# jhong93/vpd

Hardware: AMD Instinct MI355X
Metric: frame-crops/sec (VPD student train) (higher is better)
Workload: dtype bf16; 1 GPU; configs[1]: Diving48-shaped synthetic crops 128x128, ResNet-34 student (5-ch RGB+flow), emb_dim 128, sum-MSE + AdamW, batch=256 per GPU; global_batch=256, parallelism=dp1

## Files before the change

include/vpd_hip.h:

```cpp
#ifndef VPD_HIP_H
#define VPD_HIP_H
#include <stddef.h>
#ifdef __cplusplus
extern "C" {
#endif

typedef struct vpd_plan vpd_plan_t;

const char* vpd_last_error(void);
int vpd_abi_version(void);
const char* vpd_elem_dtype(void);

int vpd_plan_create(const char* arch, int c_in, int img_h, int img_w, int emb_dim, int motion,
                    int max_batch, int train, vpd_plan_t** out);
#define VPD_TRAIN_EARLY_BUCKET0 2
void vpd_plan_destroy(vpd_plan_t* plan);

int vpd_plan_num_tensors(const vpd_plan_t* plan);
int vpd_plan_tensor_info(const vpd_plan_t* plan, int i, int* kind, int* is_decoder, long long* offset,
                         long long* numel, int* ndim, int dims[4]);
long long vpd_plan_param_numel(const vpd_plan_t* plan);
int vpd_plan_num_bn(const vpd_plan_t* plan);
int vpd_plan_bn_info(const vpd_plan_t* plan, int i, int* channels, long long* rm_off, long long* rv_off);
long long vpd_plan_bn_numel(const vpd_plan_t* plan);
// ... 144 lines not shown
                            const float* gammaA, double* rowsA, void* dzA, float* dgammaA, float* dbetaA, const void* zB,
                            const float* meanB, const float* rstdB, const float* gammaB, double* rowsB, void* dzB,
                            float* dgammaB, float* dbetaB, void* sync, unsigned* err, int n, int H, int W, int C, void* stream);
int vpd_op_bn_backward_residency(int M, int C, int pair, int* out4);
int vpd_op_avgpool(const void* act_padded, int n, int H, int W, int C, int pad, float* pooled, void* stream);
int vpd_op_avgpool_bwd(const float* dpooled, int n, int H, int W, int C, void* dact, void* stream);
int vpd_op_sgemm(const float* A, const float* B, float* Y, const float* bias, int M, int N, int K, int ta, int tb, int relu,
                 void* stream);
int vpd_op_colsum(const float* A, int M, int N, float* out, void* stream);
int vpd_op_relu_mask(float* d, const float* act, long long n, void* stream);
int vpd_op_mse(const float* e, const float* t, long long n, float* de, float* loss_step, double* loss_accum, void* stream);
int vpd_op_wgrad(const void* dz_bf16, const void* x_bf16, float* dw, int n, int dzHp, int dzWp, int dzC, int dzpad,
                 int xHp, int xWp, int xC, int Hs, int Ws, int istr, int Kc, int Co, const int* tapset9,
                 float* slab, void* stream);
size_t vpd_op_wgrad_slab_bytes(void);
int vpd_op_wgrad_pair(const void* dz_bf16, const void* dz2_bf16, const void* x_bf16, float* dw, float* dw2, int n, int dzHp, int dzWp,
                      int dzC, int dzpad, int xHp, int xWp, int xC, int Hs, int Ws, int istr, int Kc, int Co, const int* tapset9,
                      float* slab, float* slab2, void* stream);
int vpd_op_wgrad_pair_lds_bytes(int Hs, int Ws, int ns, long long* bytes);
int vpd_op_tr_read_probe(const void* tile_bf16, void* out_bf16, void* stream);
size_t vpd_op_wgrad128_table_bytes(void);
size_t vpd_op_wgrad128_slab_floats(int Co, int Ci);
int vpd_op_wgrad128_group(int nprob, const void* const* dz, const void* const* x, float* const* dw, float* const* slab,
                          const int* dims, void* dev_table, void* stream);
int vpd_op_wgrad128_schedule(int n, const int* dims4, int G, int* ksplit, int* blk_begin, int* tasks, int cap,
                             double* est_us);

#ifdef __cplusplus
}
#endif
// ... 2 lines not shown
```

vpd_amd/_lib.py:

```python
import ctypes as C
import os

_HERE = os.path.dirname(os.path.abspath(__file__))
LIB_PATH = os.environ.get("VPD_LIB_PATH") or os.path.join(_HERE, "libvpdhip.so")
LIB_PATH_F16 = os.environ.get("VPD_LIB_PATH_F16") or os.path.join(_HERE, "libvpdhip_f16.so")
ABI_VERSION = 5

c_int_p = C.POINTER(C.c_int)
c_ll_p = C.POINTER(C.c_longlong)
vp = C.c_void_p

SIGNATURES = {
    "vpd_last_error": (C.c_char_p, []),
    "vpd_abi_version": (C.c_int, []),
    "vpd_elem_dtype": (C.c_char_p, []),
    "vpd_plan_create": (C.c_int, [C.c_char_p, C.c_int, C.c_int, C.c_int, C.c_int, C.c_int, C.c_int, C.c_int,
                                  C.POINTER(vp)]),
    "vpd_plan_destroy": (None, [vp]),
    "vpd_plan_num_tensors": (C.c_int, [vp]),
    "vpd_plan_tensor_info": (C.c_int, [vp, C.c_int, c_int_p, c_int_p, c_ll_p, c_ll_p, c_int_p, c_int_p]),
    "vpd_plan_param_numel": (C.c_longlong, [vp]),
    "vpd_plan_num_bn": (C.c_int, [vp]),
    "vpd_plan_bn_info": (C.c_int, [vp, C.c_int, c_int_p, c_ll_p, c_ll_p]),
    "vpd_plan_bn_numel": (C.c_longlong, [vp]),
# ... 49 lines not shown
    "vpd_op_conv1x1_bn_dispatch": (C.c_int, [C.c_int] * 6 + [c_int_p]),
    "vpd_op_stem_pool_forward": (C.c_int, [vp] * 5 + [C.c_int] * 5 + [vp]),
    "vpd_op_stem_dgrad": (C.c_int, [vp, vp, vp, C.c_int, C.c_int, C.c_int, C.c_int, vp]),
    "vpd_op_stem_pool_backward": (C.c_int, [vp] * 15 + [C.c_int] * 4 + [vp]),
    "vpd_op_bn_backward": (C.c_int, [vp] * 15 + [C.c_int] + [vp, vp] + [C.c_int] * 6 + [vp]),
    "vpd_op_bn_backward_pair": (C.c_int, [vp] * 20 + [C.c_int] * 4 + [vp]),
    "vpd_op_bn_backward_residency": (C.c_int, [C.c_int, C.c_int, C.c_int, c_int_p]),
    "vpd_op_avgpool": (C.c_int, [vp] + [C.c_int] * 5 + [vp, vp]),
    "vpd_op_avgpool_bwd": (C.c_int, [vp] + [C.c_int] * 4 + [vp, vp]),
    "vpd_op_sgemm": (C.c_int, [vp] * 4 + [C.c_int] * 6 + [vp]),
    "vpd_op_colsum": (C.c_int, [vp, C.c_int, C.c_int, vp, vp]),
    "vpd_op_relu_mask": (C.c_int, [vp, vp, C.c_longlong, vp]),
    "vpd_op_mse": (C.c_int, [vp, vp, C.c_longlong, vp, vp, vp, vp]),
    "vpd_op_wgrad": (C.c_int, [vp, vp, vp] + [C.c_int] * 13 + [c_int_p, vp, vp]),
    "vpd_op_wgrad_slab_bytes": (C.c_size_t, []),
    "vpd_op_wgrad_pair": (C.c_int, [vp] * 5 + [C.c_int] * 13 + [c_int_p, vp, vp, vp]),
    "vpd_op_wgrad_pair_lds_bytes": (C.c_int, [C.c_int, C.c_int, C.c_int, c_ll_p]),
    "vpd_op_tr_read_probe": (C.c_int, [vp, vp, vp]),
    "vpd_op_wgrad128_table_bytes": (C.c_size_t, []),
    "vpd_op_wgrad128_slab_floats": (C.c_size_t, [C.c_int, C.c_int]),
    "vpd_op_wgrad128_group": (C.c_int, [C.c_int, vp, vp, vp, vp, c_int_p, vp, vp]),
    "vpd_op_wgrad128_schedule": (C.c_int, [C.c_int, c_int_p, C.c_int, c_int_p, c_int_p, c_int_p, C.c_int,
                                           C.POINTER(C.c_double)]),
}

_libs = {}


class VpdHipError(RuntimeError):
    pass


def lib(dtype="bf16"):
    if dtype in _libs:
        return _libs[dtype]
    if dtype not in ("bf16", "fp16"):
        raise VpdHipError("unknown element type %r (bf16 | fp16)" % (dtype,))
    path = LIB_PATH if dtype == "bf16" else LIB_PATH_F16
    name = os.path.basename(path)
    if not os.path.isfile(path):
        raise VpdHipError(
            "%s not found at %s: build it with `python -c 'import __graft_entry__ as g; g.build()'` "
            "or `make -C vpd_amd/csrc`.  vpd_amd has no PyTorch/CPU fallback." % (name, path))
    import torch
    h = C.CDLL(path)
    ab_build = "VPD_LIB_PATH" in os.environ and dtype == "bf16"
    for sym, (res, args) in SIGNATURES.items():
        try:
            fn = getattr(h, sym)
        except AttributeError as e:
            if ab_build and (sym.startswith("vpd_op_") or sym in ("vpd_elem_dtype", "vpd_plan_set_loss_scale", "vpd_backward_ext")):
                continue
            raise VpdHipError("%s lacks symbol %s declared in include/vpd_hip.h" % (name, sym)) from e
        fn.restype = res
        fn.argtypes = args
    if h.vpd_abi_version() != ABI_VERSION and not (ab_build and os.environ.get("VPD_LIB_ALLOW_ABI") == str(h.vpd_abi_version())):
        raise VpdHipError("%s ABI version %d != expected %d" % (name, h.vpd_abi_version(), ABI_VERSION))
    if hasattr(h, "vpd_elem_dtype") and h.vpd_elem_dtype().decode() != dtype:
        raise VpdHipError("%s was built with %s elements, %s asked for" % (path, h.vpd_elem_dtype().decode(), dtype))
    _libs[dtype] = h
    return h
# ... 7 lines not shown
```

vpd_amd/csrc/conv_wgrad.hip:

```cpp
#include <string.h>
#include <algorithm>
#include <type_traits>
#include <utility>
#include <vector>
#include "common.h"

typedef const void __attribute__((address_space(1)))* wg_gptr_t;
typedef void __attribute__((address_space(3)))* wg_lptr_t;
typedef const char __attribute__((address_space(3)))* wg_lds_cp;

static __device__ __forceinline__ int wg_f(int r) { return ((r >> 1) & 1) | (((r >> 3) & 1) << 1); }
static __device__ __forceinline__ int wg_swz_off(int r, int col) { return r * 64 + ((((col >> 4) ^ wg_f(r)) << 4) | (col & 15)); }
static __device__ __forceinline__ int wg_src_piece(int r, int piece) { return (((piece >> 1) ^ wg_f(r)) << 1) | (piece & 1); }

static __device__ __forceinline__ bf16x8 wg_tr_read(wg_lds_cp lo_addr, wg_lds_cp hi_addr) {
    typedef s16x4 __attribute__((address_space(3))) * lds_p;
    const s16x4 lo = __builtin_amdgcn_ds_read_tr16_b64_v4i16((lds_p)lo_addr);
    const s16x4 hi = __builtin_amdgcn_ds_read_tr16_b64_v4i16((lds_p)hi_addr);
    s16x8 v;
    v[0] = lo[0]; v[1] = lo[1]; v[2] = lo[2]; v[3] = lo[3];
    v[4] = hi[0]; v[5] = hi[1]; v[6] = hi[2]; v[7] = hi[3];
    return __builtin_bit_cast(bf16x8, v);
}
static __device__ __forceinline__ bf16x8 wg_tr_read(const bf16_t* tile, int o0, int o1) {
// ... 444 lines not shown
    if (i < n4)
        for (int s2 = gi; s2 < ksplit; s2 += groups) {
            const float4 v = slab[(long)s2 * n4 + i];
            a.x += v.x; a.y += v.y; a.z += v.z; a.w += v.w;
        }
    sh[gi][o] = a;
    __syncthreads();
    if (gi == 0 && i < n4) {
        for (int k = 1; k < groups; ++k) {
            const float4 v = sh[k][o];
            a.x += v.x; a.y += v.y; a.z += v.z; a.w += v.w;
        }
        r.dw[pi][i] = a;
    }
}
static void wg_launch_reduce(const WgReduceGroup& red, hipStream_t stream) {
    if (red.nprob < 1) return;
    int max_ks = 1;
    long max_n4 = 0;
    for (int i = 0; i < red.nprob; ++i) {
        max_n4 = red.n4[i] > max_n4 ? red.n4[i] : max_n4;
        max_ks = red.ksplit[i] > max_ks ? red.ksplit[i] : max_ks;
    }
    const int groups = max_ks < 16 ? max_ks : 16;
    hipLaunchKernelGGL(wgrad_slab_reduce_group_kernel, dim3((unsigned)((max_n4 + 63) / 64), red.nprob), dim3(64 * groups), 0, stream,
                       red, groups);
}


template <int R0, int R1>
static __device__ __forceinline__ void wgrad_stem_half(const WgradParams& p, const bf16_t* ring, int STAGE, int nch,
                                                       int ctile, int lane) {
    constexpr int NT = R1 - R0;
    const int W0 = p.Ws, Wp = p.xWp;
    f32x4 acc[NT][4];
#pragma unroll
    for (int t = 0; t < NT; ++t)
#pragma unroll
        for (int a = 0; a < 4; ++a) acc[t][a] = f32x4{0.f, 0.f, 0.f, 0.f};
    const int gq = lane >> 4, i16 = lane & 15, q = i16 >> 2, pp = i16 & 3;
    int offA[4][2], baseB[2][2];
// ... 944 lines not shown
```

vpd_amd/csrc/kernels.h:

```cpp
#pragma once
#include <vector>

#include "common.h"

struct BnApplyParams {
    const bf16_t* z;
    const float* scale; const float* shift;
    int res_kind;
    const bf16_t* res; int rHp, rWp, rpad;
    const float* rscale; const float* rshift;
    bf16_t* out; int oHp, oWp, opad;
    int M, H, W, C, relu;
    unsigned char* mask_out;
    int xcd_tile_px;
};

struct StemPoolParams {
    const bf16_t* z; int Hz, Wz;
    const float* scale; const float* shift;
    bf16_t* out; int opad;
    unsigned char* idx;
    int N, Ho, Wo, C;
};

// ... 52 lines not shown
bool vpd_conv_takes_bn_sums(const ConvParams& p);
struct ConvDispatch {
    int kclass;
    int pws;
    int geo;
    int c64x2;
    int ws1x1, stream1x1;
    int halo;
    int bm, bn;
    int mode;
    int tiles_per_block;
};
ConvDispatch vpd_conv_dispatch(const ConvParams& p);
int vpd_conv_xcd_tile_px(const ConvParams& p);
hipError_t vpd_launch_wgrad_reduce(const WgradParams& p, hipStream_t stream);
extern "C" int vpd_conv_bm(int M, int Co);
hipError_t vpd_launch_wgrad(const WgradParams& p, hipStream_t stream);
size_t vpd_wgrad_slab_bytes();
bool vpd_wgrad_group_eligible(const WgradParams& p);
size_t vpd_wgrad_group_slab_floats(int M, int Co, int Kc, int ntaps = 9);
hipError_t vpd_launch_wgrad_group(const WgradParams* ps, int n, hipStream_t stream);
bool vpd_wgrad_overwrites(const WgradParams& p);
bool vpd_wgrad_pair_ok(const WgradParams& p3, const WgradParams& p1);
hipError_t vpd_launch_wgrad_pair(const WgradParams& p3, const WgradParams& p1, hipStream_t stream);
hipError_t vpd_launch_wgrad_pair_reduce(const WgradParams& p3, const WgradParams& p1, hipStream_t stream);
int vpd_wgrad_pair_lds_query(int H, int W, int ns, long long* bytes);
bool vpd_wgrad128_eligible(const WgradParams& p);
size_t vpd_wgrad128_table_bytes();
void* vpd_wgrad128_cache_new();
void vpd_wgrad128_cache_free(void* cache);
// ... 54 lines not shown
                              hipStream_t s);
hipError_t vpd_launch_avgpool_bwd(const float* dpooled, int H, int W, int C, int N, bf16_t* dact, hipStream_t s);
hipError_t vpd_launch_sgemm(const float* A, const float* B, float* Y, const float* bias, int M, int N, int K, int ta,
                            int tb, int relu, hipStream_t s);
hipError_t vpd_launch_colsum(const float* A, int M, int N, float* out, hipStream_t s);
hipError_t vpd_launch_relu_mask(float* d, const float* act, long n, hipStream_t s);
hipError_t vpd_launch_mse(const float* e, const float* t, long n, float* de, float* loss_step, double* loss_accum,
                          hipStream_t s);

hipError_t vpd_launch_pack_input(const float* x, int N, int C, int H, int W, bf16_t* out, int Hp, int Wp, int pad,
                                 int Cp, hipStream_t s);
hipError_t vpd_launch_pack_weights(const PackDesc* d_descs, int ndesc, const int* d_blockmap, int nblocks,
                                   const float* master, bf16_t* arena, hipStream_t s);
hipError_t vpd_launch_adamw_pack(const PackDesc* d_descs, const int* d_blockmap, int nblocks, float* p, const float* g,
                                 float* m, float* v, bf16_t* arena, double lr, double b1, double b2, double eps, double wd,
                                 int step, hipStream_t s, const float* wg = nullptr, float gscale = 1.f);
hipError_t vpd_launch_unpack_grads(const PackDesc* d_descs, int ndesc, const int* d_blockmap, int nblocks,
                                   const float* wg, float* grads, hipStream_t s);
hipError_t vpd_launch_adamw(float* p, const float* g, float* m, float* v, long n, double lr, double b1, double b2,
                            double eps, double wd, int step, hipStream_t s, float gscale = 1.f);
hipError_t vpd_launch_adamw_pack_scaled(const PackDesc* d_descs, const int* d_blockmap, int nblocks, float* p, const float* g,
                                        float* m, float* v, bf16_t* arena, double lr, double b1, double b2, double eps,
                                        double wd, const vpd_scale_state* st, hipStream_t s, const float* wg = nullptr);
hipError_t vpd_launch_adamw_scaled(float* p, const float* g, float* m, float* v, long n, double lr, double b1, double b2,
                                   double eps, double wd, const vpd_scale_state* st, hipStream_t s);
hipError_t vpd_launch_check_finite(const FiniteRanges& r, vpd_scale_state* st, hipStream_t s);
hipError_t vpd_launch_scale_update(vpd_scale_state* st, float growth, float backoff, int interval, hipStream_t s);
hipError_t vpd_launch_scale_by_state(float* x, long n, const vpd_scale_state* st, hipStream_t stream);

#define ZR_MAX 16
struct ZeroRanges {
    float* ptr[ZR_MAX];
    long n4[ZR_MAX];
    int count;
};
hipError_t vpd_launch_zero_ranges(const ZeroRanges& z, hipStream_t s);

struct vpd_aug_params;
// ... 10 lines not shown
```

vpd_amd/csrc/optim.hip:

```cpp
#include "../../include/vpd_hip.h"
#include "common.h"
#include "kernels.h"

template <int CT>
__global__ __launch_bounds__(256) void pack_input_kernel(const float* x, int N, int C, int H, int W, bf16_t* out,
                                                         int Hp, int Wp, int pad, int Cp) {
    const int W4 = W >> 2;
    const long total = (long)N * H * W4;
    const long plane = (long)H * W;
    const int Cn = CT ? CT : C;
    const bool fast = total < VPD_FDIV_MAX;
    const float rW4 = 1.0f / (float)W4, rH = 1.0f / (float)H;
    for (long it = (long)blockIdx.x * blockDim.x + threadIdx.x; it < total; it += (long)gridDim.x * blockDim.x) {
        int b, y, x0;
        if (fast) {
            const int q = vpd_fdiv((int)it, rW4);
            x0 = ((int)it - q * W4) << 2;
            b = vpd_fdiv(q, rH);
            y = q - b * H;
        } else {
            b = (int)(it / ((long)H * W4));
            const long r4 = it - (long)b * H * W4;
            y = (int)(r4 / W4);
            x0 = (int)(r4 - (long)y * W4) << 2;
// ... 332 lines not shown
#pragma unroll
        for (int j = 0; j < 4; ++j)
            w[j] = (unsigned int)tile[co][(q * 8 + 2 * j) * khw + tap] | ((unsigned int)tile[co][(q * 8 + 2 * j + 1) * khw + tap] << 16);
        *reinterpret_cast<uint4*>(arena + d.fwd_off + ((size_t)tap * d.Co + co0 + co) * d.Ci + ci0 + q * 8) = uint4{w[0], w[1], w[2], w[3]};
    }
    if (d.dgr_off >= 0)
        for (int i = threadIdx.x; i < 128 * khw; i += 256) {
            const int q = i & 3, ci = (i >> 2) & 31, tap = i >> 7;
            unsigned int w[4];
#pragma unroll
            for (int j = 0; j < 4; ++j)
                w[j] = (unsigned int)tile[q * 8 + 2 * j][ci * khw + tap] | ((unsigned int)tile[q * 8 + 2 * j + 1][ci * khw + tap] << 16);
            *reinterpret_cast<uint4*>(arena + d.dgr_off + ((size_t)tap * d.Ci + ci0 + ci) * d.Co + co0 + q * 8) = uint4{w[0], w[1], w[2], w[3]};
        }
}
hipError_t vpd_launch_adamw_pack(const PackDesc* d_descs, const int* d_blockmap, int nblocks, float* p, const float* g,
                                 float* m, float* v, bf16_t* arena, double lr, double b1, double b2, double eps, double wd,
                                 int step, hipStream_t s, const float* wg, float gscale) {
    if ((reinterpret_cast<size_t>(p) | reinterpret_cast<size_t>(g) | reinterpret_cast<size_t>(m) |
         reinterpret_cast<size_t>(v)) & 15)
        return hipErrorInvalidValue;
    hipLaunchKernelGGL(adamw_pack_kernel<AdamHyper>, dim3(nblocks), dim3(256), 0, s, d_descs, d_blockmap, p, g, m, v, arena,
                       adam_hyper(lr, b1, b2, eps, wd, step, gscale), wg);
    return hipGetLastError();
}
hipError_t vpd_launch_adamw_pack_scaled(const PackDesc* d_descs, const int* d_blockmap, int nblocks, float* p, const float* g,
                                        float* m, float* v, bf16_t* arena, double lr, double b1, double b2, double eps,
                                        double wd, const vpd_scale_state* st, hipStream_t s, const float* wg) {
    if ((reinterpret_cast<size_t>(p) | reinterpret_cast<size_t>(g) | reinterpret_cast<size_t>(m) |
         reinterpret_cast<size_t>(v)) & 15)
        return hipErrorInvalidValue;
    hipLaunchKernelGGL(adamw_pack_kernel<AdamHyperDyn>, dim3(nblocks), dim3(256), 0, s, d_descs, d_blockmap, p, g, m, v,
                       arena, adam_hyper_dyn(lr, b1, b2, eps, wd, st), wg);
    return hipGetLastError();
}

static __device__ __forceinline__ unsigned nonfinite1(float f) {
    return (__float_as_uint(f) & 0x7f800000u) == 0x7f800000u ? 1u : 0u;
}
static __device__ __forceinline__ unsigned nonfinite4(const float4& f) {
    return nonfinite1(f.x) | nonfinite1(f.y) | nonfinite1(f.z) | nonfinite1(f.w);
}
__global__ __launch_bounds__(256) void check_finite_kernel(const FiniteRanges r, unsigned* found) {
    __shared__ unsigned blk;
    if (threadIdx.x == 0) blk = 0u;
    __syncthreads();
// ... 72 lines not shown
```

vpd_amd/csrc/plan.h:

```cpp
#pragma once
#include <hip/hip_runtime.h>
#include <string.h>

#include <vector>

#include "../../include/vpd_hip.h"
#include "common.h"
#include "kernels.h"

int fail(const char* what, hipError_t e = hipSuccess);
#define HCHECK(expr)                                   \
    do {                                               \
        hipError_t _e = (expr);                        \
        if (_e != hipSuccess) return fail(#expr, _e);  \
    } while (0)
#define LCHECK(expr)                                   \
    do {                                               \
        hipError_t _e = (expr);                        \
        if (_e != hipSuccess) return fail(#expr, _e);  \
    } while (0)

constexpr float kBnEps = 1e-5f;
constexpr float kBnMomentum = 0.1f;

// ... 56 lines not shown
    long long nparam = 0, nparam_padded = 0, nbn = 0;
    long long arena_elems = 0, wg_elems = 0, slab_elems = 0;
    long long bucket_off[4], bucket_numel[4];
    long long bucket_wg_off[4], bucket_wg_numel[4];
    size_t ws_bytes = 0;
    size_t xin_off = 0, arena_off = 0, wg_off = 0, partial_off = 0, z0_off = 0, p0_off = 0, idx_off = 0;
    size_t g0_off = 0, dz0_off = 0, G_off[3] = {0, 0, 0}, T_off[2] = {0, 0}, slab_off = 0;
    size_t pooled_off = 0, emb_off = 0, h1_off = 0, h2_off = 0, pred_off = 0;
    size_t dpred_off = 0, dh2_off = 0, dh1_off = 0, demb_off = 0, dpooled_off = 0;
    size_t desc_off = 0, bmap_pack_off = 0, bmap_unpack_off[4] = {0, 0, 0, 0};
    int xHp = 0, xWp = 0;
    int H0 = 0, W0 = 0, H1 = 0, W1 = 0;
    std::vector<PackDesc> descs;
    std::vector<int> bmap_pack;
    std::vector<int> bmap_adam;
    size_t bmap_adam_off = 0;
    int nstem_pack_blocks = 0;
    std::vector<int> bmap_unpack[4];
    size_t partial_bytes = 0;
    struct Graph { int n; hipGraph_t g; hipGraphExec_t e; };
    std::vector<Graph> graphs;
    void* bound_ws = nullptr;
    bool fused_bn = true;
    size_t fused_off = 0, fused_bytes = 0;
    size_t syncerr_off = 0;
    bool wg_group = true;
    size_t gslab_off = 0;
    bool dgrad_sums = true;
    bool relu_bits = true;
    bool lazy_next = false, grads_in_scratch = false;
// ... 45 lines not shown
```

vpd_amd/csrc/plan.hip:

```cpp
#include <hip/hip_runtime.h>
#include <math.h>
#include <stdio.h>
#include <stdlib.h>
#include <string.h>

#include <string>
#include <algorithm>
#include <vector>

#include "plan.h"

static thread_local std::string g_err;
int fail(const char* what, hipError_t e) {
    char buf[512];
    if (e != hipSuccess) snprintf(buf, sizeof buf, "%s: %s", what, hipGetErrorString(e));
    else snprintf(buf, sizeof buf, "%s", what);
    g_err = buf;
    return -1;
}

extern "C" const char* vpd_last_error(void) { return g_err.c_str(); }
extern "C" const char* vpd_elem_dtype(void) { return VPD_ELEM_NAME; }
extern "C" int vpd_abi_version(void) { return 5; }

// ... 168 lines not shown
        };
        take(B.c1); take(B.c2);
        if (bottleneck) take(B.c3);
        if (B.ds) take(B.cd);
    }
    {
        long long at = (long long)p->stem.ntaps * p->stem.Co * p->stem.Kc;
        for (int b = 3; b >= 0; --b) {
            if (p->bucket_wg_off[b] != at) { delete p; return fail("internal: weight-gradient scratch is not bucket-contiguous"); }
            at += p->bucket_wg_numel[b];
        }
        if (at != p->wg_elems) { delete p; return fail("internal: weight-gradient scratch size mismatch"); }
    }
    {
        const int nconv = (int)p->descs.size();
        for (size_t i = 0; i + 1 < p->bmap_pack.size(); i += 2) {
            if (p->bmap_pack[i] == 0) { p->nstem_pack_blocks++; continue; }
            p->bmap_adam.push_back(p->bmap_pack[i]); p->bmap_adam.push_back(p->bmap_pack[i + 1]);
        }
        std::vector<std::pair<long long, long long>> convs;
        for (int i = 1; i < nconv; ++i)
            convs.push_back({p->descs[i].src_off, (long long)p->descs[i].Co * p->descs[i].Ci * p->descs[i].kh * p->descs[i].kw});
        std::sort(convs.begin(), convs.end());
        long long pos = 0;
        auto plain = [&](long long a, long long b) {
            if (b <= a) return;
            PackDesc d = {};
            d.src_off = a; d.numel = b - a; d.stem = 2; d.kh = d.kw = 1; d.dgr_off = -1;
            const int id = (int)p->descs.size();
            p->descs.push_back(d);
            for (long long ch = 0; ch * 2048 < b - a; ++ch) { p->bmap_adam.push_back(id); p->bmap_adam.push_back((int)ch); }
        };
        for (auto& cv : convs) { plain(pos, cv.first); pos = cv.first + cv.second; }
        plain(pos, p->nparam_padded);
// ... 305 lines not shown

extern "C" int vpd_plan_adamw_step(vpd_plan_t* p, float* params, const float* grads, float* adam_m, float* adam_v,
                                   long long numel, double lr, double beta1, double beta2, double eps,
                                   double weight_decay, int step, void* workspace, void* stream) {
    if (!p || !params || !grads || !adam_m || !adam_v || !workspace) return fail("null argument");
    if (p->bound_ws != workspace) return fail("workspace not initialised with vpd_plan_init_workspace");
    if (numel % 4 || numel < p->nparam_padded) return fail("numel must be a multiple of 4 and cover the plan's parameters");
    if (step < 1) return fail("step is 1-based");
    hipStream_t s = (hipStream_t)stream;
    char* ws = (char*)workspace;
    LCHECK(vpd_launch_adamw_pack(reinterpret_cast<const PackDesc*>(ws + p->desc_off),
                                 reinterpret_cast<const int*>(ws + p->bmap_adam_off), (int)p->bmap_adam.size() / 2, params,
                                 grads, adam_m, adam_v, reinterpret_cast<bf16_t*>(ws + p->arena_off), lr, beta1, beta2,
                                 eps, weight_decay, step, s,
                                 p->grads_in_scratch ? reinterpret_cast<const float*>(ws + p->wg_off) : nullptr,
                                 1.0f / p->loss_scale));
    p->grads_in_scratch = false;
    LCHECK(vpd_launch_pack_weights(reinterpret_cast<const PackDesc*>(ws + p->desc_off), (int)p->descs.size(),
                                   reinterpret_cast<const int*>(ws + p->bmap_pack_off), p->nstem_pack_blocks, params,
                                   reinterpret_cast<bf16_t*>(ws + p->arena_off), s));
    if (numel > p->nparam_padded)
        LCHECK(vpd_launch_adamw(params + p->nparam_padded, grads + p->nparam_padded, adam_m + p->nparam_padded,
                                adam_v + p->nparam_padded, (long)(numel - p->nparam_padded), lr, beta1, beta2, eps,
                                weight_decay, step, s, 1.0f / p->loss_scale));
    return 0;
}

extern "C" int vpd_plan_set_loss_scale(vpd_plan_t* p, float scale) {
    if (!p) return fail("null plan");
    if (!(scale > 0.f) || !(scale < 3.0e38f)) return fail("loss scale must be a positive finite number");
    p->loss_scale = scale;
// ... 71 lines not shown
    return 0;
}

extern "C" int vpd_plan_adamw_step_scaled(vpd_plan_t* p, float* params, const float* grads, float* adam_m, float* adam_v,
                                          long long numel, double lr, double beta1, double beta2, double eps,
                                          double weight_decay, const vpd_scale_state* state, void* workspace, void* stream) {
    if (!p || !params || !grads || !adam_m || !adam_v || !state || !workspace) return fail("null argument");
    if (p->bound_ws != workspace) return fail("workspace not initialised with vpd_plan_init_workspace");
    if (numel % 4 || numel < p->nparam_padded) return fail("numel must be a multiple of 4 and cover the plan's parameters");
    hipStream_t s = (hipStream_t)stream;
    char* ws = (char*)workspace;
    LCHECK(vpd_launch_adamw_pack_scaled(reinterpret_cast<const PackDesc*>(ws + p->desc_off),
                                        reinterpret_cast<const int*>(ws + p->bmap_adam_off), (int)p->bmap_adam.size() / 2,
                                        params, grads, adam_m, adam_v, reinterpret_cast<bf16_t*>(ws + p->arena_off), lr, beta1,
                                        beta2, eps, weight_decay, state, s,
                                        p->grads_in_scratch ? reinterpret_cast<const float*>(ws + p->wg_off) : nullptr));
    p->grads_in_scratch = false;
    LCHECK(vpd_launch_pack_weights(reinterpret_cast<const PackDesc*>(ws + p->desc_off), (int)p->descs.size(),
                                   reinterpret_cast<const int*>(ws + p->bmap_pack_off), p->nstem_pack_blocks, params,
                                   reinterpret_cast<bf16_t*>(ws + p->arena_off), s));
    if (numel > p->nparam_padded)
        LCHECK(vpd_launch_adamw_scaled(params + p->nparam_padded, grads + p->nparam_padded, adam_m + p->nparam_padded,
                                       adam_v + p->nparam_padded, (long)(numel - p->nparam_padded), lr, beta1, beta2, eps,
                                       weight_decay, state, s));
    return 0;
}

extern "C" int vpd_scale_state_update(vpd_scale_state* state, float growth, float backoff, int growth_interval, void* stream) {
    if (!state) return fail("null argument");
    if (!(growth >= 1.f) || !(growth < 3.0e38f)) return fail("growth factor must be finite and >= 1");
    if (!(backoff > 0.f) || !(backoff <= 1.f)) return fail("backoff factor must be in (0, 1]");
// ... 48 lines not shown
    for (auto& t : p->timed) {
        HCHECK(hipEventSynchronize(t.b));
        float ms = 0.f;
        HCHECK(hipEventElapsedTime(&ms, t.a, t.b));
        const int cls = t.cls;
        p->ev_pool.push_back(t.a); p->ev_pool.push_back(t.b);
        if (cls < 0 || cls >= nclasses) continue;
        out[3 * cls + 0] += 1.0; out[3 * cls + 1] += ms; out[3 * cls + 2] += t.flops;
    }
    p->timed.clear();
    return 0;
}

extern "C" int vpd_op_conv_bm(int M, int Co) { return vpd_conv_bm(M, Co); }
extern "C" size_t vpd_op_wgrad_slab_bytes(void) { return vpd_wgrad_slab_bytes(); }

static TapSet tapset_from(const int* t) {
    TapSet ts;
    ts.nr = t[0]; ts.nc = t[1]; ts.dy0 = t[2]; ts.dys = t[3]; ts.dx0 = t[4]; ts.dxs = t[5];
    ts.w0 = t[6]; ts.wrs = t[7]; ts.wcs = t[8];
    return ts;
}

extern "C" int vpd_op_conv2d(const void* x, const void* w, void* y, double* stats, int n, int xHp, int xWp, int xC,
                             int yHp, int yWp, int yC, int ypad, int Hs, int Ws, int osub, int oph, int opw, int istr,
                             int Kc, int Co, const int* tapset9, int accumulate, void* stream) {
    ConvParams q;
    memset(&q, 0, sizeof q);
    q.x = (const bf16_t*)x; q.xHp = xHp; q.xWp = xWp; q.xC = xC; q.w = (const bf16_t*)w;
    q.y = (bf16_t*)y; q.yHp = yHp; q.yWp = yWp; q.yC = yC; q.ypad = ypad; q.stats = stats;
// ... 453 lines not shown
```

vpd_amd/csrc/switches.h:

```cpp
#pragma once
#include <stdlib.h>

#define VPD_SWITCHES(X)                                        \
    X(fused_bn,           "VPD_FUSED_BN",          1)          \
    X(bn_pair,            "VPD_BN_PAIR",           1)          \
    X(bn_xcd,             "VPD_BN_XCD",            1)          \
    X(bn_xcd_force,       "VPD_BN_XCD_FORCE",     -1)          \
    X(dgrad_sums,         "VPD_DGRAD_SUMS",        1)          \
    X(dgrad_sums_l1,      "VPD_DGRAD_SUMS_L1",     1)          \
    X(dgrad_sums_s2,      "VPD_DGRAD_SUMS_S2",     1)          \
    X(dgrad_sums_pair,    "VPD_DGRAD_SUMS_PAIR",   1)          \
    X(dgrad_sums_1x1,     "VPD_DGRAD_SUMS_1X1",    1)          \
    X(relu_bits,          "VPD_RELU_BITS",         1)          \
    X(poolbwd_fold,       "VPD_POOLBWD_FOLD",      1)          \
    X(ds_merge,           "VPD_DS_MERGE",          1)          \
    X(pws,                "VPD_PWS",               1)          \
    X(pws_blocks,         "VPD_PWS_BLOCKS",        0)          \
    X(ws_256x64,          "VPD_WS_256x64",         1)          \
    X(ws_mw8,             "VPD_WS_MW8",            1)          \
    X(no_ws,              "VPD_NO_WS",             0)          \
    X(pws_geo,            "VPD_PWS_GEO",           1)          \
    X(pws_rot,            "VPD_PWS_ROT",           1)          \
    X(reserve_cus,        "VPD_RESERVE_CUS",       0)          \
    X(c64x2,              "VPD_C64X2",             1)          \
    X(conv1x1_ws,         "VPD_CONV1X1_WS",        1)          \
    X(conv_s2_ws,         "VPD_CONV_S2_WS",        1)          \
    X(conv_s2_dgrad_ws,   "VPD_CONV_S2_DGRAD_WS",  1)          \
    X(wg2,                "VPD_WG2",               1)          \
    X(wg2_1x1,            "VPD_WG2_1X1",           1)          \
    X(wg2_tco256,         "VPD_WG2_TCO256",        1)          \
    X(conv1x1_stream,     "VPD_CONV1X1_STREAM",    1)          \
    X(bneck_recompute,    "VPD_BNECK_RECOMPUTE",   1)          \
    X(wg_group,           "VPD_WG_GROUP",          1)          \
    X(wg_merge,           "VPD_WG_MERGE",          1)          \
    X(wgrad_1x1,          "VPD_WGRAD_1X1",        -1)          \
    X(wgrad_s2,           "VPD_WGRAD_S2",          1)          \
    X(wgrad_ds_ride,      "VPD_WGRAD_DS_RIDE",     1)          \
    X(stem_lds_store,     "VPD_STEM_LDS_STORE",    1)          \
    X(stem_pair,          "VPD_STEM_PAIR",         1)          \
    X(stem_quad,          "VPD_STEM_QUAD",         1)          \
    X(stem_poolsums,      "VPD_STEM_POOLSUMS",     1)          \
    X(stem_pool_fused,    "VPD_STEM_POOL_FUSED",   1)          \
    X(ablate,             "VPD_ABLATE",            0)

struct VpdSwitches {
#define VPD_SWITCH_FIELD(field, env, dflt) int field;
    VPD_SWITCHES(VPD_SWITCH_FIELD)
#undef VPD_SWITCH_FIELD
};

inline const VpdSwitches& vpd_switches() {
    static const VpdSwitches s = [] {
// ... 9 lines not shown
```

Baseline: 78510 crops/s.

## Add multi-row wgrad slab reduce and 64-wide tiled AdamW pack kernel

Adds a wgrad split-K slab reduction kernel in which each block reduces several 64-float4 rows at once. The row count is chosen so the grid still fills the CU budget, which cuts block count and per-block overhead for large weight tensors. It also adds an AdamW+pack kernel that processes 32x64 weight tiles with 576 threads, transposing scratch-layout gradients through LDS and writing both forward and dgrad bf16 arenas from one tile. Both are on by default behind switches, and the tiled AdamW path falls back if any conv has shapes it cannot handle. It also adds test entry points (a list reduce, a reduce logger and an input-pack op) and fixes f16 library-path detection.

```diff
diff --git a/include/vpd_hip.h b/include/vpd_hip.h
--- a/include/vpd_hip.h
+++ b/include/vpd_hip.h
@@ -182,6 +182,10 @@
                  int xHp, int xWp, int xC, int Hs, int Ws, int istr, int Kc, int Co, const int* tapset9,
                  float* slab, void* stream);
 size_t vpd_op_wgrad_slab_bytes(void);
+int vpd_op_wgrad_reduce(int nprob, const float* const* slabs, float* const* dws, const long long* nfloats, const int* ksplits,
+                        int variant, void* stream);
+int vpd_op_wgrad_reduce_log(long long* out, int cap);
+int vpd_op_pack_input(const float* x, int n, int c, int H, int W, void* out, int Hp, int Wp, int pad, int variant, void* stream);
 int vpd_op_wgrad_pair(const void* dz_bf16, const void* dz2_bf16, const void* x_bf16, float* dw, float* dw2, int n, int dzHp, int dzWp,
                       int dzC, int dzpad, int xHp, int xWp, int xC, int Hs, int Ws, int istr, int Kc, int Co, const int* tapset9,
                       float* slab, float* slab2, void* stream);
diff --git a/vpd_amd/_lib.py b/vpd_amd/_lib.py
--- a/vpd_amd/_lib.py
+++ b/vpd_amd/_lib.py
@@ -87,6 +87,9 @@
     "vpd_op_mse": (C.c_int, [vp, vp, C.c_longlong, vp, vp, vp, vp]),
     "vpd_op_wgrad": (C.c_int, [vp, vp, vp] + [C.c_int] * 13 + [c_int_p, vp, vp]),
     "vpd_op_wgrad_slab_bytes": (C.c_size_t, []),
+    "vpd_op_wgrad_reduce": (C.c_int, [C.c_int, C.POINTER(vp), C.POINTER(vp), c_ll_p, c_int_p, C.c_int, vp]),
+    "vpd_op_wgrad_reduce_log": (C.c_int, [c_ll_p, C.c_int]),
+    "vpd_op_pack_input": (C.c_int, [vp, C.c_int, C.c_int, C.c_int, C.c_int, vp, C.c_int, C.c_int, C.c_int, C.c_int, vp]),
     "vpd_op_wgrad_pair": (C.c_int, [vp] * 5 + [C.c_int] * 13 + [c_int_p, vp, vp, vp]),
     "vpd_op_wgrad_pair_lds_bytes": (C.c_int, [C.c_int, C.c_int, C.c_int, c_ll_p]),
     "vpd_op_tr_read_probe": (C.c_int, [vp, vp, vp]),
@@ -117,7 +120,7 @@
             "or `make -C vpd_amd/csrc`.  vpd_amd has no PyTorch/CPU fallback." % (name, path))
     import torch
     h = C.CDLL(path)
-    ab_build = "VPD_LIB_PATH" in os.environ and dtype == "bf16"
+    ab_build = ("VPD_LIB_PATH" if dtype == "bf16" else "VPD_LIB_PATH_F16") in os.environ
     for sym, (res, args) in SIGNATURES.items():
         try:
             fn = getattr(h, sym)
diff --git a/vpd_amd/csrc/conv_wgrad.hip b/vpd_amd/csrc/conv_wgrad.hip
--- a/vpd_amd/csrc/conv_wgrad.hip
+++ b/vpd_amd/csrc/conv_wgrad.hip
@@ -1,5 +1,6 @@
 #include <string.h>
 #include <algorithm>
+#include <mutex>
 #include <type_traits>
 #include <utility>
 #include <vector>
@@ -482,8 +483,71 @@
         r.dw[pi][i] = a;
     }
 }
-static void wg_launch_reduce(const WgReduceGroup& red, hipStream_t stream) {
+template <int ROWS>
+__global__ __launch_bounds__(1024) void wgrad_slab_reduce_rows_kernel(const WgReduceGroup r, int groups) {
+    extern __shared__ __attribute__((aligned(16))) unsigned char wg_reduce_smem[];
+    float4 (*sh)[64] = reinterpret_cast<float4 (*)[64]>(wg_reduce_smem);
+    const int pi = blockIdx.y;
+    const long n4 = r.n4[pi];
+    const int ksplit = r.ksplit[pi];
+    const float4* __restrict__ slab = r.slab[pi];
+    const int o = threadIdx.x & 63, gi = threadIdx.x >> 6;
+    const long i0 = (long)blockIdx.x * (64 * ROWS) + o;
+    if ((long)blockIdx.x * (64 * ROWS) >= n4) return;
+    long ic[ROWS];
+    float4 a[ROWS];
+#pragma unroll
+    for (int u = 0; u < ROWS; ++u) {
+        const long i = i0 + u * 64;
+        ic[u] = i < n4 ? i : n4 - 1;
+        a[u] = float4{0.f, 0.f, 0.f, 0.f};
+    }
+    for (int s2 = gi; s2 < ksplit; s2 += groups) {
+        float4 v[ROWS];
+#pragma unroll
+        for (int u = 0; u < ROWS; ++u) v[u] = slab[(long)s2 * n4 + ic[u]];
+#pragma unroll
+        for (int u = 0; u < ROWS; ++u) { a[u].x += v[u].x; a[u].y += v[u].y; a[u].z += v[u].z; a[u].w += v[u].w; }
+    }
+#pragma unroll
+    for (int u = 0; u < ROWS; ++u) sh[gi * ROWS + u][o] = a[u];
+    __syncthreads();
+    for (int u = gi; u < ROWS; u += groups) {
+        const long i = i0 + u * 64;
+        if (i >= n4) break;
+        float4 t = sh[u][o];
+#pragma unroll 4
+        for (int k = 1; k < groups; ++k) {
+            const float4 v = sh[k * ROWS + u][o];
+            t.x += v.x; t.y += v.y; t.z += v.z; t.w += v.w;
+        }
+        r.dw[pi][i] = t;
+    }
+}
+#ifdef VPD_ENABLE_ABLATE
+static struct { std::mutex mu; bool on = false; std::vector<long long> rec; } wg_reduce_log;
+static void wg_reduce_log_add(const WgReduceGroup& red) {
+    std::lock_guard<std::mutex> lk(wg_reduce_log.mu);
+    if (!wg_reduce_log.on) return;
+    wg_reduce_log.rec.push_back(red.nprob);
+    for (int i = 0; i < red.nprob; ++i) { wg_reduce_log.rec.push_back(red.n4[i] * 4); wg_reduce_log.rec.push_back(red.ksplit[i]); }
+}
+int vpd_wgrad_reduce_log(long long* out, int cap) {
+    std::lock_guard<std::mutex> lk(wg_reduce_log.mu);
+    if (!out) { wg_reduce_log.on = true; wg_reduce_log.rec.clear(); return 0; }
+    wg_reduce_log.on = false;
+    size_t n = 0;
+    const std::vector<long long>& r = wg_reduce_log.rec;
+    while (n < r.size() && n + 1 + 2 * (size_t)r[n] <= (size_t)(cap < 0 ? 0 : cap)) n += 1 + 2 * (size_t)r[n];
+    if (n) memcpy(out, r.data(), n * sizeof(long long));
+    return (int)n;
+}
+#endif
+static void wg_launch_reduce(const WgReduceGroup& red, hipStream_t stream, int variant = -1) {
     if (red.nprob < 1) return;
+#ifdef VPD_ENABLE_ABLATE
+    wg_reduce_log_add(red);
+#endif
     int max_ks = 1;
     long max_n4 = 0;
     for (int i = 0; i < red.nprob; ++i) {
@@ -491,8 +555,35 @@
         max_ks = red.ksplit[i] > max_ks ? red.ksplit[i] : max_ks;
     }
     const int groups = max_ks < 16 ? max_ks : 16;
-    hipLaunchKernelGGL(wgrad_slab_reduce_group_kernel, dim3((unsigned)((max_n4 + 63) / 64), red.nprob), dim3(64 * groups), 0, stream,
-                       red, groups);
+    if (variant < 0) variant = vpd_switches().wg_reduce_rows;
+    int rows = variant ? (groups <= 4 ? 8 : 4) : 1;
+    for (; rows > 1; rows >>= 1) {
+        long blocks = 0;
+        for (int i = 0; i < red.nprob; ++i) blocks += (red.n4[i] + 64 * rows - 1) / (64 * rows);
+        if (blocks >= vpd_cu_budget()) break;
+    }
+    if (rows == 1) {
+        hipLaunchKernelGGL(wgrad_slab_reduce_group_kernel, dim3((unsigned)((max_n4 + 63) / 64), red.nprob), dim3(64 * groups), 0, stream,
+                           red, groups);
+        return;
+    }
+    const dim3 grid((unsigned)((max_n4 + 64 * rows - 1) / (64 * rows)), red.nprob), block(64 * groups);
+    const size_t lds = (size_t)groups * rows * 64 * sizeof(float4);
+    if (rows == 8) hipLaunchKernelGGL(wgrad_slab_reduce_rows_kernel<8>, grid, block, lds, stream, red, groups);
+    else if (rows == 4) hipLaunchKernelGGL(wgrad_slab_reduce_rows_kernel<4>, grid, block, lds, stream, red, groups);
+    else hipLaunchKernelGGL(wgrad_slab_reduce_rows_kernel<2>, grid, block, lds, stream, red, groups);
+}
+hipError_t vpd_launch_wgrad_reduce_list(int nprob, const float* const* slabs, float* const* dws, const long long* nfloats,
+                                        const int* ksplits, int variant, hipStream_t stream) {
+    if (nprob < 1 || nprob > WG_GROUP_MAX) return hipErrorInvalidValue;
+    WgReduceGroup red = {};
+    for (int i = 0; i < nprob; ++i) {
+        if (!slabs[i] || !dws[i] || nfloats[i] < 4 || nfloats[i] % 4 || ksplits[i] < 1) return hipErrorInvalidValue;
+        if ((reinterpret_cast<size_t>(slabs[i]) | reinterpret_cast<size_t>(dws[i])) & 15) return hipErrorInvalidValue;
+        red.add(slabs[i], dws[i], (long)nfloats[i], ksplits[i]);
+    }
+    wg_launch_reduce(red, stream, variant);
+    return hipGetLastError();
 }
 
 
diff --git a/vpd_amd/csrc/kernels.h b/vpd_amd/csrc/kernels.h
--- a/vpd_amd/csrc/kernels.h
+++ b/vpd_amd/csrc/kernels.h
@@ -90,6 +90,11 @@
 ConvDispatch vpd_conv_dispatch(const ConvParams& p);
 int vpd_conv_xcd_tile_px(const ConvParams& p);
 hipError_t vpd_launch_wgrad_reduce(const WgradParams& p, hipStream_t stream);
+#ifdef VPD_ENABLE_ABLATE
+int vpd_wgrad_reduce_log(long long* out, int cap);
+#endif
+hipError_t vpd_launch_wgrad_reduce_list(int nprob, const float* const* slabs, float* const* dws, const long long* nfloats,
+                                        const int* ksplits, int variant, hipStream_t stream);
 extern "C" int vpd_conv_bm(int M, int Co);
 hipError_t vpd_launch_wgrad(const WgradParams& p, hipStream_t stream);
 size_t vpd_wgrad_slab_bytes();
@@ -174,14 +179,16 @@
                                    const float* master, bf16_t* arena, hipStream_t s);
 hipError_t vpd_launch_adamw_pack(const PackDesc* d_descs, const int* d_blockmap, int nblocks, float* p, const float* g,
                                  float* m, float* v, bf16_t* arena, double lr, double b1, double b2, double eps, double wd,
-                                 int step, hipStream_t s, const float* wg = nullptr, float gscale = 1.f);
+                                 int step, hipStream_t s, const float* wg = nullptr, float gscale = 1.f,
+                                 bool tile64 = false);
 hipError_t vpd_launch_unpack_grads(const PackDesc* d_descs, int ndesc, const int* d_blockmap, int nblocks,
                                    const float* wg, float* grads, hipStream_t s);
 hipError_t vpd_launch_adamw(float* p, const float* g, float* m, float* v, long n, double lr, double b1, double b2,
                             double eps, double wd, int step, hipStream_t s, float gscale = 1.f);
 hipError_t vpd_launch_adamw_pack_scaled(const PackDesc* d_descs, const int* d_blockmap, int nblocks, float* p, const float* g,
                                         float* m, float* v, bf16_t* arena, double lr, double b1, double b2, double eps,
-                                        double wd, const vpd_scale_state* st, hipStream_t s, const float* wg = nullptr);
+                                        double wd, const vpd_scale_state* st, hipStream_t s, const float* wg = nullptr,
+                                        bool tile64 = false);
 hipError_t vpd_launch_adamw_scaled(float* p, const float* g, float* m, float* v, long n, double lr, double b1, double b2,
                                    double eps, double wd, const vpd_scale_state* st, hipStream_t s);
 hipError_t vpd_launch_check_finite(const FiniteRanges& r, vpd_scale_state* st, hipStream_t s);
diff --git a/vpd_amd/csrc/optim.hip b/vpd_amd/csrc/optim.hip
--- a/vpd_amd/csrc/optim.hip
+++ b/vpd_amd/csrc/optim.hip
@@ -370,22 +370,149 @@
             *reinterpret_cast<uint4*>(arena + d.dgr_off + ((size_t)tap * d.Ci + ci0 + ci) * d.Co + co0 + q * 8) = uint4{w[0], w[1], w[2], w[3]};
         }
 }
+#define ADAM64_THREADS 576
+template <bool SCRATCH>
+static __device__ __forceinline__ void adamw_tile64_3x3(const PackDesc& d, int co0, int ci0, float* __restrict__ p,
+                                                        const float* __restrict__ g, float* __restrict__ m, float* __restrict__ v,
+                                                        const float* __restrict__ wgc, const AdamHyper& h,
+                                                        unsigned short (*tile)[64 * 9 + 2], float (*gs)[4 * 576]) {
+    const int t = threadIdx.x;
+    const int r = t / 144, w = t - r * 144;
+    const int k = w << 2;
+    const int gtap = w >> 4, gc = (w & 15) << 2;
+    float4 pn, mn, vn, gn;
+    auto load = [&](int s) {
+        const size_t e = d.src_off + ((size_t)(co0 + 4 * s + r) * d.Ci + ci0) * 9 + k;
+        pn = *reinterpret_cast<const float4*>(p + e);
+        mn = *reinterpret_cast<const float4*>(m + e);
+        vn = *reinterpret_cast<const float4*>(v + e);
+        gn = SCRATCH ? *reinterpret_cast<const float4*>(wgc + ((size_t)gtap * d.Co + co0 + 4 * s + r) * d.Kc + ci0 + gc)
+                     : *reinterpret_cast<const float4*>(g + e);
+    };
+    load(0);
+#pragma unroll
+    for (int s = 0; s < 8; ++s) {
+        float4 pp = pn, mm = mn, vv = vn, gg = gn;
+        const size_t e = d.src_off + ((size_t)(co0 + 4 * s + r) * d.Ci + ci0) * 9 + k;
+        if (SCRATCH) {
+            float* q = gs[s & 1] + r * 576 + gc * 9 + gtap;
+            q[0] = gg.x; q[9] = gg.y; q[18] = gg.z; q[27] = gg.w;
+            __syncthreads();
+        }
+        if (s + 1 < 8) load(s + 1);
+        if (SCRATCH) gg = *reinterpret_cast<const float4*>(gs[s & 1] + r * 576 + k);
+        adamw4(pp, gg, mm, vv, h);
+        *reinterpret_cast<float4*>(p + e) = pp;
+        *reinterpret_cast<float4*>(m + e) = mm;
+        *reinterpret_cast<float4*>(v + e) = vv;
+        unsigned* tw = reinterpret_cast<unsigned*>(&tile[4 * s + r][k]);
+        tw[0] = (unsigned)f2bf(pp.x) | ((unsigned)f2bf(pp.y) << 16);
+        tw[1] = (unsigned)f2bf(pp.z) | ((unsigned)f2bf(pp.w) << 16);
+    }
+}
+template <class H>
+__global__ __launch_bounds__(ADAM64_THREADS) void adamw_tile64_kernel(const PackDesc* __restrict__ descs, const int* __restrict__ blockmap,
+                                                                      float* __restrict__ p, const float* __restrict__ g,
+                                                                      float* __restrict__ m, float* __restrict__ v,
+                                                                      bf16_t* __restrict__ arena, const H hh, const float* __restrict__ wg) {
+    __shared__ __attribute__((aligned(16))) unsigned short tile[32][64 * 9 + 2];
+    __shared__ __attribute__((aligned(16))) float gs[2][4 * 576];
+    bool live;
+    const AdamHyper h = adam_live(hh, live);
+    if (!live) return;
+    const PackDesc d = descs[blockmap[2 * blockIdx.x]];
+    const int chunk = blockmap[2 * blockIdx.x + 1];
+    const int t = threadIdx.x;
+    if (d.stem == 2) {
+        const long e0 = d.src_off + (long)chunk * ADAM_PLAIN_CHUNK;
+        const long e1 = d.src_off + d.numel;
+        const long end = e0 + ADAM_PLAIN_CHUNK < e1 ? e0 + ADAM_PLAIN_CHUNK : e1;
+        const long n4 = (e0 & 3) ? 0 : (end - e0) >> 2;
+        if (t < n4) {
+            const long e = e0 + 4 * t;
+            float4 pp = *reinterpret_cast<const float4*>(p + e), mm = *reinterpret_cast<const float4*>(m + e);
+            float4 vv = *reinterpret_cast<const float4*>(v + e);
+            adamw4(pp, *reinterpret_cast<const float4*>(g + e), mm, vv, h);
+            *reinterpret_cast<float4*>(p + e) = pp;
+            *reinterpret_cast<float4*>(m + e) = mm;
+            *reinterpret_cast<float4*>(v + e) = vv;
+        }
+        for (long e = e0 + 4 * n4 + t; e < end; e += ADAM64_THREADS) {
+            float pp = p[e], mm = m[e], vv = v[e];
+            adamw1(pp, g[e], mm, vv, h);
+            p[e] = pp; m[e] = mm; v[e] = vv;
+        }
+        return;
+    }
+    const int khw = d.kh * d.kw;
+    const int tci = d.Ci >> 6;
+    const int co0 = (chunk / tci) * 32, ci0 = (chunk % tci) * 64;
+    const float* wgc = wg ? wg + d.wg_off : nullptr;
+    if (khw == 9) {
+        if (wgc) adamw_tile64_3x3<true>(d, co0, ci0, p, g, m, v, wgc, h, tile, gs);
+        else adamw_tile64_3x3<false>(d, co0, ci0, p, g, m, v, wgc, h, tile, gs);
+    } else if (t < 512) {
+        const int r = t >> 4, k = (t & 15) << 2;
+        const size_t e = d.src_off + (size_t)(co0 + r) * d.Ci + ci0 + k;
+        float4 pp = *reinterpret_cast<const float4*>(p + e), mm = *reinterpret_cast<const float4*>(m + e);
+        float4 vv = *reinterpret_cast<const float4*>(v + e);
+        const float4 gg = wgc ? *reinterpret_cast<const float4*>(wgc + (size_t)(co0 + r) * d.Kc + ci0 + k)
+                              : *reinterpret_cast<const float4*>(g + e);
+        adamw4(pp, gg, mm, vv, h);
+        *reinterpret_cast<float4*>(p + e) = pp;
+        *reinterpret_cast<float4*>(m + e) = mm;
+        *reinterpret_cast<float4*>(v + e) = vv;
+        unsigned* tw = reinterpret_cast<unsigned*>(&tile[r][k]);
+        tw[0] = (unsigned)f2bf(pp.x) | ((unsigned)f2bf(pp.y) << 16);
+        tw[1] = (unsigned)f2bf(pp.z) | ((unsigned)f2bf(pp.w) << 16);
+    }
+    __syncthreads();
+    for (int i = t; i < 256 * khw; i += ADAM64_THREADS) {
+        const int q = i & 7, co = (i >> 3) & 31, tap = i >> 8;
+        unsigned int w4[4];
+#pragma unroll
+        for (int j = 0; j < 4; ++j)
+            w4[j] = (unsigned int)tile[co][(q * 8 + 2 * j) * khw + tap] | ((unsigned int)tile[co][(q * 8 + 2 * j + 1) * khw + tap] << 16);
+        *reinterpret_cast<uint4*>(arena + d.fwd_off + ((size_t)tap * d.Co + co0 + co) * d.Ci + ci0 + q * 8) = uint4{w4[0], w4[1], w4[2], w4[3]};
+    }
+    if (d.dgr_off >= 0)
+        for (int i = t; i < 256 * khw; i += ADAM64_THREADS) {
+            const int q = i & 3, ci = (i >> 2) & 63, tap = i >> 8;
+            unsigned int w4[4];
+#pragma unroll
+            for (int j = 0; j < 4; ++j)
+                w4[j] = (unsigned int)tile[q * 8 + 2 * j][ci * khw + tap] | ((unsigned int)tile[q * 8 + 2 * j + 1][ci * khw + tap] << 16);
+            *reinterpret_cast<uint4*>(arena + d.dgr_off + ((size_t)tap * d.Ci + ci0 + ci) * d.Co + co0 + q * 8) = uint4{w4[0], w4[1], w4[2], w4[3]};
+        }
+}
 hipError_t vpd_launch_adamw_pack(const PackDesc* d_descs, const int* d_blockmap, int nblocks, float* p, const float* g,
                                  float* m, float* v, bf16_t* arena, double lr, double b1, double b2, double eps, double wd,
-                                 int step, hipStream_t s, const float* wg, float gscale) {
+                                 int step, hipStream_t s, const float* wg, float gscale, bool tile64) {
     if ((reinterpret_cast<size_t>(p) | reinterpret_cast<size_t>(g) | reinterpret_cast<size_t>(m) |
          reinterpret_cast<size_t>(v)) & 15)
         return hipErrorInvalidValue;
+    if (tile64) {
+        if (reinterpret_cast<size_t>(wg) & 15) return hipErrorInvalidValue;
+        hipLaunchKernelGGL(adamw_tile64_kernel<AdamHyper>, dim3(nblocks), dim3(ADAM64_THREADS), 0, s, d_descs, d_blockmap, p, g, m, v,
+                           arena, adam_hyper(lr, b1, b2, eps, wd, step, gscale), wg);
+        return hipGetLastError();
+    }
     hipLaunchKernelGGL(adamw_pack_kernel<AdamHyper>, dim3(nblocks), dim3(256), 0, s, d_descs, d_blockmap, p, g, m, v, arena,
                        adam_hyper(lr, b1, b2, eps, wd, step, gscale), wg);
     return hipGetLastError();
 }
 hipError_t vpd_launch_adamw_pack_scaled(const PackDesc* d_descs, const int* d_blockmap, int nblocks, float* p, const float* g,
                                         float* m, float* v, bf16_t* arena, double lr, double b1, double b2, double eps,
-                                        double wd, const vpd_scale_state* st, hipStream_t s, const float* wg) {
+                                        double wd, const vpd_scale_state* st, hipStream_t s, const float* wg, bool tile64) {
     if ((reinterpret_cast<size_t>(p) | reinterpret_cast<size_t>(g) | reinterpret_cast<size_t>(m) |
          reinterpret_cast<size_t>(v)) & 15)
         return hipErrorInvalidValue;
+    if (tile64) {
+        if (reinterpret_cast<size_t>(wg) & 15) return hipErrorInvalidValue;
+        hipLaunchKernelGGL(adamw_tile64_kernel<AdamHyperDyn>, dim3(nblocks), dim3(ADAM64_THREADS), 0, s, d_descs, d_blockmap, p, g, m, v,
+                           arena, adam_hyper_dyn(lr, b1, b2, eps, wd, st), wg);
+        return hipGetLastError();
+    }
     hipLaunchKernelGGL(adamw_pack_kernel<AdamHyperDyn>, dim3(nblocks), dim3(256), 0, s, d_descs, d_blockmap, p, g, m, v,
                        arena, adam_hyper_dyn(lr, b1, b2, eps, wd, st), wg);
     return hipGetLastError();
diff --git a/vpd_amd/csrc/plan.h b/vpd_amd/csrc/plan.h
--- a/vpd_amd/csrc/plan.h
+++ b/vpd_amd/csrc/plan.h
@@ -94,6 +94,7 @@
     std::vector<PackDesc> descs;
     std::vector<int> bmap_pack;
     std::vector<int> bmap_adam;
+    bool adam_tile64 = false;
     size_t bmap_adam_off = 0;
     int nstem_pack_blocks = 0;
     std::vector<int> bmap_unpack[4];
diff --git a/vpd_amd/csrc/plan.hip b/vpd_amd/csrc/plan.hip
--- a/vpd_amd/csrc/plan.hip
+++ b/vpd_amd/csrc/plan.hip
@@ -206,10 +206,19 @@
     }
     {
         const int nconv = (int)p->descs.size();
+        p->adam_tile64 = vpd_switches().adamw_tile64 != 0;
+        for (int i = 1; i < nconv; ++i) {
+            const PackDesc& d = p->descs[i];
+            if (d.Ci % 64 || d.Co % 32 || d.kh != d.kw || (d.kh != 3 && d.kh != 1)) p->adam_tile64 = false;
+        }
         for (size_t i = 0; i + 1 < p->bmap_pack.size(); i += 2) {
             if (p->bmap_pack[i] == 0) { p->nstem_pack_blocks++; continue; }
+            if (p->adam_tile64) continue;
             p->bmap_adam.push_back(p->bmap_pack[i]); p->bmap_adam.push_back(p->bmap_pack[i + 1]);
         }
+        if (p->adam_tile64)
+            for (int i = 1; i < nconv; ++i)
+                for (int ch = 0; ch < (p->descs[i].Co / 32) * (p->descs[i].Ci / 64); ++ch) { p->bmap_adam.push_back(i); p->bmap_adam.push_back(ch); }
         std::vector<std::pair<long long, long long>> convs;
         for (int i = 1; i < nconv; ++i)
             convs.push_back({p->descs[i].src_off, (long long)p->descs[i].Co * p->descs[i].Ci * p->descs[i].kh * p->descs[i].kw});
@@ -545,7 +554,7 @@
                                  grads, adam_m, adam_v, reinterpret_cast<bf16_t*>(ws + p->arena_off), lr, beta1, beta2,
                                  eps, weight_decay, step, s,
                                  p->grads_in_scratch ? reinterpret_cast<const float*>(ws + p->wg_off) : nullptr,
-                                 1.0f / p->loss_scale));
+                                 1.0f / p->loss_scale, p->adam_tile64));
     p->grads_in_scratch = false;
     LCHECK(vpd_launch_pack_weights(reinterpret_cast<const PackDesc*>(ws + p->desc_off), (int)p->descs.size(),
                                    reinterpret_cast<const int*>(ws + p->bmap_pack_off), p->nstem_pack_blocks, params,
@@ -647,7 +656,8 @@
                                         reinterpret_cast<const int*>(ws + p->bmap_adam_off), (int)p->bmap_adam.size() / 2,
                                         params, grads, adam_m, adam_v, reinterpret_cast<bf16_t*>(ws + p->arena_off), lr, beta1,
                                         beta2, eps, weight_decay, state, s,
-                                        p->grads_in_scratch ? reinterpret_cast<const float*>(ws + p->wg_off) : nullptr));
+                                        p->grads_in_scratch ? reinterpret_cast<const float*>(ws + p->wg_off) : nullptr,
+                                        p->adam_tile64));
     p->grads_in_scratch = false;
     LCHECK(vpd_launch_pack_weights(reinterpret_cast<const PackDesc*>(ws + p->desc_off), (int)p->descs.size(),
                                    reinterpret_cast<const int*>(ws + p->bmap_pack_off), p->nstem_pack_blocks, params,
@@ -726,6 +736,30 @@
 
 extern "C" int vpd_op_conv_bm(int M, int Co) { return vpd_conv_bm(M, Co); }
 extern "C" size_t vpd_op_wgrad_slab_bytes(void) { return vpd_wgrad_slab_bytes(); }
+extern "C" int vpd_op_wgrad_reduce(int nprob, const float* const* slabs, float* const* dws, const long long* nfloats,
+                                   const int* ksplits, int variant, void* stream) {
+    if (!slabs || !dws || !nfloats || !ksplits) return fail("null argument");
+    if (variant < -1 || variant > 1) return fail("variant must be -1, 0 or 1");
+    LCHECK(vpd_launch_wgrad_reduce_list(nprob, slabs, dws, nfloats, ksplits, variant, (hipStream_t)stream));
+    return 0;
+}
+extern "C" int vpd_op_wgrad_reduce_log(long long* out, int cap) {
+#ifdef VPD_ENABLE_ABLATE
+    return vpd_wgrad_reduce_log(out, cap);
+#else
+    (void)out; (void)cap;
+    return fail("vpd_op_wgrad_reduce_log: the recorder is compiled in with -DVPD_ENABLE_ABLATE only");
+#endif
+}
+extern "C" int vpd_op_pack_input(const float* x, int n, int c, int H, int W, void* out, int Hp, int Wp, int pad, int variant,
+                                 void* stream) {
+    if (!x || !out) return fail("null argument");
+    if (n < 1 || c < 1 || c > 8 || H < 1 || W < 1 || pad < 0 || Hp < H + 2 * pad || Wp < W + 2 * pad) return fail("bad shape");
+    if (variant != -1 && variant != 0) return fail("input packing has one kernel per shape: variant must be -1 or 0");
+    if (reinterpret_cast<size_t>(out) & 15) return fail("out must be 16-byte aligned");
+    LCHECK(vpd_launch_pack_input(x, n, c, H, W, (bf16_t*)out, Hp, Wp, pad, 8, (hipStream_t)stream));
+    return 0;
+}
 
 static TapSet tapset_from(const int* t) {
     TapSet ts;
diff --git a/vpd_amd/csrc/switches.h b/vpd_amd/csrc/switches.h
--- a/vpd_amd/csrc/switches.h
+++ b/vpd_amd/csrc/switches.h
@@ -36,6 +36,8 @@
     X(wgrad_1x1,          "VPD_WGRAD_1X1",        -1)          \
     X(wgrad_s2,           "VPD_WGRAD_S2",          1)          \
     X(wgrad_ds_ride,      "VPD_WGRAD_DS_RIDE",     1)          \
+    X(wg_reduce_rows,     "VPD_WG_REDUCE_ROWS",    1)          \
+    X(adamw_tile64,       "VPD_ADAMW_TILE64",      1)          \
     X(stem_lds_store,     "VPD_STEM_LDS_STORE",    1)          \
     X(stem_pair,          "VPD_STEM_PAIR",         1)          \
     X(stem_quad,          "VPD_STEM_QUAD",         1)          \
```

New measurement: 79220 crops/s, median of 6. About the same (+0.9%).
